# parthjaggi/flow

Measured on AMD Instinct MI355X. Metric: env-steps/sec, higher is better.
Workload: dtype mixed

## Files before the change

flow_amd/csrc/flowsim.hip:

```cpp
#include "flowsim_sim.h"
#include "flowsim_learn.h"
#include "flowsim_es.h"

#include <cmath>

namespace fsim {

int validate(const fs_config* c) {
  if (!c) return fail(FS_ERR_INVALID, "fs_create: cfg is NULL");
  if (c->struct_size != sizeof(fs_config))
    return fail(FS_ERR_INVALID, "fs_create: struct_size mismatch (header/library out of sync)");
  if (c->abi_version != FS_ABI_VERSION) return fail(FS_ERR_INVALID, "fs_create: abi_version mismatch");
  if (c->precision != FS_F32 && c->precision != FS_F64 && c->precision != FS_MIXED && c->precision != FS_F16S)
    return fail(FS_ERR_INVALID, "fs_create: bad precision");
  if (c->precision == FS_F16S && (c->network != FS_NET_MERGE || c->num_vehicles > 64))
    return fail(FS_ERR_UNSUPPORTED, "fs_create: FS_F16S (half state, float32 integrator) is built for FS_NET_MERGE "
                                    "(k_steps_open, <= 64 vehicle slots)");
  if (c->precision == FS_MIXED && (c->network == FS_NET_MERGE || c->network == FS_NET_BOTTLENECK)) {
  } else if (c->precision == FS_MIXED) {
    const bool fig8 = c->network == FS_NET_FIGURE_EIGHT;
    const char* why = nullptr;
    if ((c->network != FS_NET_RING && !fig8) || c->num_lanes > 1) why = "network (single-lane ring or figure eight)";
    else if (c->env == FS_ENV_MULTI_WAVE_ATTENUATION_PO)
      why = "env (FS_ENV_MULTI_WAVE_ATTENUATION_PO is built for FS_F32, and for FS_F64 on the generic kernel)";
// ... 251 lines not shown
  s->seg = seg;
  hipError_t e = hipSetDevice(cfg->device);
  if (e == hipSuccess) e = hipStreamCreateWithFlags(&s->own_stream, hipStreamNonBlocking);
  if (e != hipSuccess) {
    delete s;
    return fail(FS_ERR_HIP, std::string("fs_create: no usable HIP device: ") + hipGetErrorString(e));
  }
  s->stream = s->own_stream;
  {
    const std::pair<const char*, bool SimBase::*> switches[] = {
        {"FLOWSIM_FORCE_GENERIC", &SimBase::force_generic}, {"FLOWSIM_NO_FASTDIV", &SimBase::no_fastdiv},
        {"FLOWSIM_NO_LOOP_KERNEL", &SimBase::no_loop_kernel}, {"FLOWSIM_NO_LOOP_FULL", &SimBase::no_loop_full},
        {"FLOWSIM_NO_RING_RL", &SimBase::no_ring_rl}, {"FLOWSIM_NO_QUEUE", &SimBase::no_queue},
        {"FLOWSIM_NO_PAIR", &SimBase::no_pair}, {"FLOWSIM_PAIR_GENERIC_N", &SimBase::pair_generic_n},
        {"FLOWSIM_KERNEL_DETAIL", &SimBase::kernel_detail}, {"FLOWSIM_PAIR_N_ALWAYS", &SimBase::pair_n_always},
        {"FLOWSIM_NO_MASK_SKIP", &SimBase::no_mask_skip},
        {"FLOWSIM_SNAPSHOT_COPIES", &SimBase::snap_copies}};
    for (const auto& sw : switches) {
      const char* v = std::getenv(sw.first);
      s->*sw.second = v && v[0] == '1';
    }
  }
  int rc = s->init();
  if (rc == FS_OK) {
    hipError_t e2 = hipStreamSynchronize(s->stream);
    if (e2 != hipSuccess) rc = fail(FS_ERR_HIP, std::string("fs_create: ") + hipGetErrorString(e2));
  }
  if (rc != FS_OK) {
    for (void* p : s->allocs) (void)hipFree(p);
    (void)hipStreamDestroy(s->own_stream);
// ... 779 lines not shown
```

flow_amd/csrc/flowsim_launch.h:

```cpp
#pragma once
#include "flowsim_sim.h"
#ifdef FS_PART_QUEUE
#include "flowsim_queue.h"
#include "flowsim_dropq.h"
#endif

namespace fsim {

#ifdef FS_PART_QUEUE
  template <typename T>
  int Sim<T>::launch_queue(const StepArgs& a) {
    const bool po = dv.env == FS_ENV_MERGE_PO;
    const bool noise = (dv.flags & fs::FLAG_HAS_NOISE) != 0, act = a.actions != nullptr && (po || ov.ma_apply_actions != 0);
    const auto k = pick(noise, [&](auto NZ) {
      return pick(act, [&](auto ACT) {
        return pick(po, [&](auto PO) { return &fs::k_merge_queue<NZ, ACT, false, PO>; });
      });
    });
    last_kernel = "k_merge_queue";
    hipLaunchKernelGGL(k, dim3(dv.R), dim3(64), 0, stream, dv, ov, qc, a.num_steps, a.actions, a.act_stride, a.obs, a.rew,
                       a.done, a.obs_every_step, fs::PolicyView{}, static_cast<float*>(nullptr), static_cast<float*>(nullptr),
                       0);
    return launched();
  }
// ... 159 lines not shown
  int Sim<T>::launch_obs_mixed(const StepArgs& a) {
    if constexpr (std::is_same<T, double>::value) {
      const int n = dv.R * dv.N;
      last_kernel = "k_obs_mixed";
      hipLaunchKernelGGL((fs::k_obs_mixed<T>), dim3((n + 255) / 256), dim3(256), 0, stream, dv, a.obs);
      return launched();
    } else {
      return fail(FS_ERR_UNSUPPORTED, "k_obs_mixed is a float64 kernel");
    }
  }

  template <typename T>
  template <int SEG>
  int Sim<T>::launch_pair(const StepArgs& a) {
    constexpr int ROW = SEG >= 16 ? SEG / 2 : 8;
    const bool fd = fastdiv_ok(), bc = neg_speed_possible, sm = speed_mode_any;
    const bool noise = std::is_same<T, float>::value && (dv.flags & fs::FLAG_HAS_NOISE);
    auto clamped = [&](auto SM, auto NZ) {
      return delta4 && fd && !bc ? &fs::k_rollout_pair<T, ROW, true, true, false, SM, NZ>
                                 : &fs::k_rollout_pair<T, ROW, false, false, true, SM, NZ>;
    };
    decltype(&fs::k_rollout_pair<T, ROW, false, false, true>) k = nullptr;
    if (noise) {
      if constexpr (std::is_same<T, float>::value) k = pick(sm, [&](auto SM) { return clamped(SM, std::true_type()); });
    } else if (sm) {
      k = clamped(std::true_type(), std::false_type());
    } else {
      k = pick(bc, [&](auto BC) {
        return delta4 && fd ? &fs::k_rollout_pair<T, ROW, true, true, BC>
                            : delta4 ? &fs::k_rollout_pair<T, ROW, true, false, BC> : &fs::k_rollout_pair<T, ROW, false, false, BC>;
      });
    }
    last_kernel = noise ? (sm ? "k_rollout_pair+speed_mode+noise" : "k_rollout_pair+noise")
                        : (sm ? "k_rollout_pair+speed_mode" : "k_rollout_pair");
    const int waves = (dv.R + (64 / ROW) - 1) / (64 / ROW);
    if constexpr (SEG == 32) {
      if (dv.N == 22 && delta4 && fd && !bc && !pair_generic_n && (a.num_steps >= PAIR_N_MIN_STEPS || pair_n_always)) {
        decltype(&fs::k_rollout_pair_n<T, 11>) kn = nullptr;
        if constexpr (std::is_same<T, float>::value) {
          kn = pick(sm, [&](auto SM) { return pick(noise, [&](auto NZ) { return &fs::k_rollout_pair_n<T, 11, SM, NZ>; }); });
        } else {
          kn = pick(sm, [&](auto SM) { return &fs::k_rollout_pair_n<T, 11, SM>; });
        }
        if (kernel_detail)
          last_kernel = noise ? (sm ? "k_rollout_pair+speed_mode+noise[n11]" : "k_rollout_pair+noise[n11]")
                              : (sm ? "k_rollout_pair+speed_mode[n11]" : "k_rollout_pair[n11]");
        hipLaunchKernelGGL(kn, dim3((waves + 3) / 4), dim3(256), 0, stream, dv, a.num_steps, a.obs, a.rew, a.done);
        return launched();
      }
    }
    hipLaunchKernelGGL(k, dim3((waves + 3) / 4), dim3(256), 0, stream, dv, a.num_steps, a.obs, a.rew, a.done);
    return launched();
  }

  template <typename T>
  template <int SEG>
  int Sim<T>::launch_idm(const StepArgs& a) {
    constexpr int RPW = 64 / SEG;
    const bool fd = fastdiv_ok();
    const auto k = pick(neg_speed_possible, [&](auto BC) {
      return delta4 && fd ? &fs::k_rollout_idm<T, SEG, true, true, BC>
                          : delta4 ? &fs::k_rollout_idm<T, SEG, true, false, BC> : &fs::k_rollout_idm<T, SEG, false, false, BC>;
    });
    last_kernel = "k_rollout_idm";
    const int waves = (dv.R + RPW - 1) / RPW;
    hipLaunchKernelGGL(k, dim3((waves + 7) / 8), dim3(512), 0, stream, dv, a.num_steps, a.obs, a.rew, a.done, d_dump);
    return launched();
// ... 125 lines not shown
```

flow_amd/csrc/flowsim_pair.h:

```cpp
#pragma once
#include "flowsim_kernels.h"

namespace fs {

typedef float f2 __attribute__((ext_vector_type(2)));
typedef unsigned u2v __attribute__((__vector_size__(8)));

enum : int { DPP_ROW_NEWBCAST0 = 0x150, DPP_ROW_NEWBCAST8 = 0x158 };

__device__ __forceinline__ f2 fma2(f2 a, f2 b, f2 c) { return __builtin_elementwise_fma(a, b, c); }
__device__ __forceinline__ f2 splat(float a) { return f2{a, a}; }

__device__ __forceinline__ f2 pk_mul(f2 a, f2 b) { return a * b; }
__device__ __forceinline__ f2 pk_add(f2 a, f2 b) { return a + b; }
__device__ __forceinline__ f2 pk_sub(f2 a, f2 b) { return a - b; }
__device__ __forceinline__ f2 pk_fma(f2 a, f2 b, f2 c) { return fma2(a, b, c); }
__device__ __forceinline__ f2 pk_fnma(f2 a, f2 b, f2 c) { return fma2(-a, b, c); }
__device__ __forceinline__ float nonneg_else(float x, float y) {
  const unsigned a = __builtin_bit_cast(unsigned, x), b = __builtin_bit_cast(unsigned, y);
  return __builtin_bit_cast(float, min(a, b));
}

template <int ROW>
__device__ __forceinline__ float next_a(float v, bool last, int lane) {
// ... 149 lines not shown
      "v_fma_f64 v[130:131], -v[134:135], %[ms], v[130:131]\n"
      "v_fma_f64 v[132:133], -v[136:137], %[ms], v[132:133]\n"
      "v_fma_f64 v[134:135], v[130:131], %[rcms], v[134:135]\n"
      "v_fma_f64 v[136:137], v[132:133], %[rcms], v[136:137]\n"
      "v_cvt_f32_f64_e32 v128, v[134:135]\n"
      "v_cvt_f32_f64_e32 v129, v[136:137]\n"
      : "+{v[112:113]}"(V), "+{v[114:115]}"(X), "+{v[116:117]}"(H), "+{v[118:119]}"(DVL), "={v[128:129]}"(OV),
        [cb] "+v"(crash_bits), [sq] "=&v"(sq)
      : [L2] "v"(c.L2), [lenlead] "v"(c.len_lead), [gap2] "v"(c.gap2), [vmask] "v"(c.vmask), [tvm] "v"(c.tvm),
        [ms] "v"(c.ms64), [rcms] "v"(c.rc_ms64), [last] "s"(c.last_mask)
      : "v124", "v125", "v126", "v127", "v130", "v131", "v132", "v133", "v134", "v135", "v136", "v137");
}

struct MixedConsts {
  f2 p0, p1, p2, p5, rc_v0, tsab, rc_ab, one, gap2, vmask, tvm;
  float c1e3;
  double dt, ramp, L, rc_L, rc_ms, len_b, len_next, zero;
  unsigned L_lo, L_hi, thr;
  unsigned long long last_mask;
};
__device__ __forceinline__ void mixed_step_asm_a(f2& V32, double& XA, double& XB, double& VA, double& VB, f2& H, f2& DVL,
                                                 f2& OV, const MixedConsts& c) {
  asm volatile(
      "v_pk_mul_f32 v[124:125], v[112:113], v[142:143]\n"
      "v_pk_mul_f32 v[126:127], v[124:125], %[rcab]\n"
      "v_pk_fma_f32 v[130:131], v[126:127], %[tsab], v[124:125] neg_lo:[1,0,0] neg_hi:[1,0,0]\n"
      "v_pk_fma_f32 v[126:127], v[130:131], %[rcab], v[126:127]\n"
      "v_pk_mul_f32 v[124:125], v[112:113], %[rcv0]\n"
      "v_rcp_f32_e32 v122, v140\n"
      "v_rcp_f32_e32 v123, v141\n"
      "v_pk_fma_f32 v[130:131], v[124:125], %[p0], v[112:113] neg_lo:[1,0,0] neg_hi:[1,0,0]\n"
// ... 148 lines not shown
      "v_mul_f64 v[122:123], v[138:139], %[rcms]\n"
      "v_cvt_f32_f64_e32 v128, v[120:121]\n"
      "v_cvt_f32_f64_e32 v129, v[122:123]\n"
      : "+{v[112:113]}"(V32), "+{v[114:115]}"(XA), "+{v[116:117]}"(XB), "+{v[118:119]}"(VA), "+{v[138:139]}"(VB),
        "+{v[140:141]}"(H), "+{v[142:143]}"(DVL), "={v[128:129]}"(OV)
      : [c1e3] "v"(c.c1e3), [rcab] "v"(c.rc_ab), [tsab] "v"(c.tsab), [rcv0] "v"(c.rc_v0), [p0] "v"(c.p0),
        [p1] "v"(c.p1), [p2] "v"(c.p2), [p5] "v"(c.p5), [one] "v"(c.one), [dt] "v"(c.dt), [ramp] "v"(c.ramp),
        [rcms] "v"(c.rc_ms), [zero] "v"(c.zero), [rcts] "v"(m.rc_ts), [ts] "v"(m.ts),
        [rcsm] "v"(m.rc_smax), [smax] "v"(m.smax), [tau] "v"(m.tau), [mgap] "v"(m.min_gap), [maxa] "v"(m.maxa),
        [fl0a] "v"(d.fl0a), [fl0b] "v"(d.fl0b), [adta] "v"(d.adta), [adtb] "v"(d.adtb), [ddta] "v"(d.ddta),
        [ddtb] "v"(d.ddtb)
      : "v120", "v121", "v122", "v123", "v124", "v125", "v126", "v127", "v130", "v131", "v132", "v133", "v134",
        "v135", "v136", "v137", "v146", "v147", "v148", "v149", "v150", "v151", "v152", "v153", "v154", "v155");
}
__device__ __forceinline__ void mixed_step_asm_b(f2& V32, double& XA, double& XB, f2& H, f2& DVL, f2& OX, const double& WA,
                                                 const double& WB, float& ct, float& sq, unsigned long long& need,
                                                 const MixedConsts& c) {
  asm volatile(
      "v_sub_f32_e32 v142, v112, v113\n"
      "v_subrev_f32_dpp v143, v112, v113 row_shl:1 row_mask:0xf bank_mask:0xf bound_ctrl:1\n"
      "v_subrev_f32_dpp v124, v112, v113 row_newbcast:0 row_mask:0xf bank_mask:0xf\n"
      "v_mov_b32_dpp v130, v114 row_shl:1 row_mask:0xf bank_mask:0xf bound_ctrl:1\n"
      "v_mov_b32_dpp v131, v115 row_shl:1 row_mask:0xf bank_mask:0xf bound_ctrl:1\n"
      "v_mov_b32_dpp v132, v114 row_newbcast:0 row_mask:0xf bank_mask:0xf\n"
      "v_mov_b32_dpp v133, v115 row_newbcast:0 row_mask:0xf bank_mask:0xf\n"
      "v_add_f64 v[134:135], v[116:117], -v[114:115]\n"
      "v_cndmask_b32_e64 v130, v130, v132, %[last]\n"
      "v_cndmask_b32_e64 v131, v131, v133, %[last]\n"
      "v_add_f64 v[134:135], v[134:135], %[wa]\n"
      "v_add_f64 v[136:137], v[130:131], -v[116:117]\n"
      "v_cndmask_b32_e64 v143, v143, v124, %[last]\n"
      "v_add_f64 v[120:121], v[134:135], -%[lenb]\n"
      "v_add_f64 v[136:137], v[136:137], %[wb]\n"
      "v_max3_u32 v126, v115, v117, v135\n"
      "v_add_f64 v[122:123], v[136:137], -%[lennext]\n"
      "v_cvt_f32_f64_e32 v140, v[120:121]\n"
      "v_cvt_f32_f64_e32 v141, v[122:123]\n"
      "v_min_f32_e32 v127, v140, v141\n"
      "v_sub_u32_e32 v125, v127, %[c1e3]\n"
      "v_max3_u32 v126, v126, v137, v125\n"
      "v_cmp_le_u32_e64 %[need], %[thr], v126\n"
      "v_mul_f64 v[120:121], v[114:115], %[rcL]\n"
      "v_mul_f64 v[122:123], v[116:117], %[rcL]\n"
      "v_pk_fma_f32 v[124:125], v[112:113], %[vmask], %[tvm]\n"
      "v_cvt_f32_f64_e32 v144, v[120:121]\n"
      "v_cvt_f32_f64_e32 v145, v[122:123]\n"
      "v_pk_mul_f32 v[124:125], v[124:125], v[124:125]\n"
      "v_sub_f32_e32 %[ct], v127, %[gap]\n"
      "v_add_f32_e32 %[sq], v124, v125\n"
      : "+{v[112:113]}"(V32), "+{v[114:115]}"(XA), "+{v[116:117]}"(XB), "+{v[140:141]}"(H), "+{v[142:143]}"(DVL),
        "=&{v[144:145]}"(OX), [ct] "=&v"(ct), [sq] "=&v"(sq), [need] "=&s"(need)
      : [wa] "{v[156:157]}"(WA), [wb] "{v[158:159]}"(WB), [rcL] "v"(c.rc_L), [gap] "v"(c.gap2.x), [vmask] "v"(c.vmask), [tvm] "v"(c.tvm),
        [lenb] "v"(c.len_b), [lennext] "v"(c.len_next), [c1e3] "v"(c.c1e3), [thr] "v"(c.thr), [last] "s"(c.last_mask)
      : "v120", "v121", "v122", "v123", "v124", "v125", "v126", "v127", "v130", "v131", "v132", "v133", "v134", "v135",
        "v136", "v137");
}
__device__ __forceinline__ void mixed_step_asm_slow(double& XA, double& XB, f2& H, f2& OX, double& WA, double& WB, float& ct,
                                                    const MixedConsts& c) {
  unsigned long long sa, sb;
  asm volatile(
      "v_add_f64 v[134:135], v[114:115], -%[L]\n"
      "v_add_f64 v[136:137], v[116:117], -%[L]\n"
      "v_cmp_gt_i32_e64 %[sa], 0, v135\n"
      "v_cmp_gt_i32_e64 %[sb], 0, v137\n"
      "s_nop 0\n"
      "v_cndmask_b32_e64 v114, v134, v114, %[sa]\n"
      "v_cndmask_b32_e64 v115, v135, v115, %[sa]\n"
      "v_cndmask_b32_e64 v116, v136, v116, %[sb]\n"
// ... 21 lines not shown
      "v_add_f64 v[134:135], v[134:135], -%[lenb]\n"
      "v_cvt_f32_f64_e32 v140, v[134:135]\n"
      "v_cndmask_b32_e64 v136, v136, v132, %[sb]\n"
      "v_cndmask_b32_e64 v137, v137, v133, %[sb]\n"
      "v_cndmask_b32_e64 v158, 0, %[Llo], %[sb]\n"
      "v_cndmask_b32_e64 v159, 0, %[Lhi], %[sb]\n"
      "v_add_f64 v[136:137], v[136:137], -%[lennext]\n"
      "v_cvt_f32_f64_e32 v141, v[136:137]\n"
      "v_pk_add_f32 v[126:127], v[140:141], %[gap2] neg_lo:[0,1] neg_hi:[0,1]\n"
      "v_cmp_nlt_f32_e64 %[sa], |v140|, %[c1e3]\n"
      "v_cmp_nlt_f32_e64 %[sb], |v141|, %[c1e3]\n"
      "v_min_f32_e32 %[ct], v126, v127\n"
      "v_cndmask_b32_e64 v140, %[c1e3], v140, %[sa]\n"
      "v_cndmask_b32_e64 v141, %[c1e3], v141, %[sb]\n"
      : "+{v[114:115]}"(XA), "+{v[116:117]}"(XB), "+{v[140:141]}"(H), "+{v[144:145]}"(OX), "+{v[156:157]}"(WA),
        "+{v[158:159]}"(WB), [ct] "+v"(ct), [sa] "=&s"(sa), [sb] "=&s"(sb)
      : [L] "v"(c.L), [Llo] "v"(c.L_lo), [Lhi] "v"(c.L_hi), [rcL] "v"(c.rc_L), [gap2] "v"(c.gap2), [lenb] "v"(c.len_b),
        [lennext] "v"(c.len_next), [c1e3] "v"(c.c1e3), [last] "s"(c.last_mask)
      : "v120", "v121", "v122", "v123", "v126", "v127", "v130", "v131", "v132", "v133", "v134", "v135", "v136", "v137");
}

template <typename F, int... S>
__device__ __forceinline__ void each_slot(F&& f, std::integer_sequence<int, S...>) {
  (f(std::integral_constant<int, S>()), ...);
}

template <typename T, int ROW, bool DELTA4, bool FASTDIV, bool BADCHK, bool SM, bool NOISE, int NH>
__device__ __forceinline__ void rollout_pair_body(const DevView<T>& s, int num_steps, float* __restrict__ obs,
                                                  float* __restrict__ rew, uint8_t* __restrict__ done) {
  constexpr bool MIXED = sizeof(T) == 8;
  static_assert(!(NOISE && MIXED), "FS_MIXED has no noise form (its C twin cannot reproduce the hardware's log / cos)");
// ... 32 lines not shown
      gauss4<float>(s.seed_lo, s.seed_hi, s.rep0 + uint32_t(rr), uint32_t(iA), nctr >> 2, gA, s.noise_exact != 0);
      gauss4<float>(s.seed_lo, s.seed_hi, s.rep0 + uint32_t(rr), uint32_t(iB), nctr >> 2, gB, s.noise_exact != 0);
      for (uint32_t q = 0; q < (nctr & 3u); ++q) {
        gA[0] = gA[1]; gA[1] = gA[2]; gA[2] = gA[3];
        gB[0] = gB[1]; gB[1] = gB[2]; gB[2] = gB[3];
      }
    }
  }

  const float dt = float(s.dt), ramp = float(s.ramp);
  const f2 two_sqrt_ab = {2.0f * tsqrt(p[2].x * p[3].x), 2.0f * tsqrt(p[2].y * p[3].y)};
  const f2 rc_v0 = {1.0f / p[0].x, 1.0f / p[0].y}, rc_ab = {1.0f / two_sqrt_ab.x, 1.0f / two_sqrt_ab.y};
  const float Lf = float(L);
  const f2 L2 = splat(Lf), rc_L2 = splat(1.0f / Lf), one = splat(1.0f), dt2 = splat(dt), ramp2 = splat(ramp);
  const f2 gap2 = splat(float(s.crash_gap)), m100 = splat(-100.0f);
  const f2 vmask = splat(valid ? 1.0f : 0.0f), tvm = splat(valid ? -float(s.target_velocity) : 0.0f);
  const double ms64 = double(s.max_speed), rc_ms64 = 1.0 / ms64;
  const double L64 = double(L), rc_L64 = 1.0 / L64, dt64 = double(s.dt), ramp64 = double(s.ramp);

  f2 x, v;
  double xdA = 0, xdB = 0, vdA = 0, vdB = 0;
  if (MIXED) {
    xdA = double(s.pos[idx]); xdB = double(s.pos[idx + 1]);
    vdA = double(s.vel[idx]); vdB = double(s.vel[idx + 1]);
    v = f2{float(vdA), float(vdB)};
    x = f2{0.0f, 0.0f};
  } else {
    x = f2{float(s.pos[idx]), float(s.pos[idx + 1])};
    v = f2{float(s.vel[idx]), float(s.vel[idx + 1])};
  }
  const f2 len_lead = {float(lenB), float(len_nextA)};
// ... 18 lines not shown
  f2 vl = {v.y, next_a<ROW>(v.x, last, lane)};
  f2 dvl = v - vl;
  PairConsts pc;
  pc.p0 = p[0]; pc.p1 = p[1]; pc.p2 = p[2]; pc.p5 = p[5]; pc.rc_v0 = rc_v0; pc.tsab = two_sqrt_ab; pc.rc_ab = rc_ab;
  pc.one = one; pc.dt2 = dt2; pc.ramp2 = ramp2; pc.L2 = L2; pc.rc_L2 = rc_L2; pc.len_lead = len_lead;
  pc.gap2 = gap2; pc.vmask = vmask; pc.tvm = tvm; pc.c1e3 = 1e-3f; pc.ms64 = ms64; pc.rc_ms64 = rc_ms64;
  pc.last_mask = __ballot(last);
  MixedConsts mc;
  mc.p0 = p[0]; mc.p1 = p[1]; mc.p2 = p[2]; mc.p5 = p[5]; mc.rc_v0 = rc_v0; mc.tsab = two_sqrt_ab; mc.rc_ab = rc_ab;
  mc.one = one; mc.gap2 = gap2; mc.vmask = vmask; mc.tvm = tvm; mc.c1e3 = 1e-3f; mc.dt = dt64; mc.ramp = ramp64;
  mc.L = L64; mc.rc_L = rc_L64; mc.rc_ms = rc_ms64; mc.len_b = double(lenB); mc.len_next = double(len_nextA);
  mc.zero = 0.0; mc.last_mask = pc.last_mask;
  {
    const unsigned long long Lb = __builtin_bit_cast(unsigned long long, L64);
    mc.L_lo = unsigned(Lb); mc.L_hi = unsigned(Lb >> 32);
    mc.thr = mc.L_hi < 0x457CED91u ? mc.L_hi : 0x457CED91u;
  }
  double wA = 0.0, wB = 0.0;
  if constexpr (ASM && MIXED) {
    asm volatile("" : "+v"(mc.dt), "+v"(mc.ramp), "+v"(mc.one), "+v"(mc.zero), "+v"(mc.rc_ms), "+v"(mc.c1e3), "+v"(mc.gap2));
    const double xn = next_a<ROW>(xdA, last, lane);
    wA = xdB - xdA < 0.0 ? L64 : 0.0;
    wB = xn - xdB < 0.0 ? L64 : 0.0;
    h.x = tabs(h.x) < 1e-3f ? 1e-3f : h.x;
    h.y = tabs(h.y) < 1e-3f ? 1e-3f : h.y;
  }
  SumoPair sc{};
  double floor0A = 0, floor0B = 0, adtA = 0, adtB = 0, ddtA = 0, ddtB = 0;
  if constexpr (SM) {
    const int mA = s.speed_mode[iA], mB = s.speed_mode[iB];
    const float maA = float(s.max_accel[iA]), maB = float(s.max_accel[iB]);
    const float mdA = float(s.max_decel[iA]), mdB = float(s.max_decel[iB]);
    sc.tau = f2{float(s.sumo_tau[iA]), float(s.sumo_tau[iB])};
    sc.min_gap = f2{float(s.sumo_min_gap[iA]), float(s.sumo_min_gap[iB])};
    sc.maxa = f2{maA, maB};
// ... 101 lines not shown
        if (fresh) {
          gauss4<float>(s.seed_lo, s.seed_hi, s.rep0 + uint32_t(rr), uint32_t(iA), nctr >> 2, gA, s.noise_exact != 0);
          gauss4<float>(s.seed_lo, s.seed_hi, s.rep0 + uint32_t(rr), uint32_t(iB), nctr >> 2, gB, s.noise_exact != 0);
        }
      }
      const float tA = sigma.x * gA[0], tB = sigma.y * gB[0];
      nz.x = noisyA ? tA : -0.0f;
      nz.y = noisyB ? tB : -0.0f;
      gA[0] = gA[1]; gA[1] = gA[2]; gA[2] = gA[3];
      gB[0] = gB[1]; gB[1] = gB[2]; gB[2] = gB[3];
      nctr += 1u;
    }
    return nz;
  };

  auto one_step = [&](int slot, __amdgpu_buffer_rsrc_t rs, float& sq_out, auto IN_RING, __amdgpu_buffer_rsrc_t rs_prev)
                      __attribute__((always_inline)) {
    if constexpr (ASM) {
      f2 ov, ox;
      const unsigned so = unsigned(slot) * step_b32;
      auto store_late = [&]() {
        if constexpr (decltype(IN_RING)::value) {
          if (!BURST && slot >= 1 && slot <= NPIECE) __builtin_amdgcn_raw_buffer_store_b128(piece, rs_prev, doff[slot - 1], 0, 0);
        } else {
          if (slot > 0) __builtin_amdgcn_raw_buffer_store_b128(piece, rs, off_16, so - step_b32, 0);
        }
      };
      auto rows_in = [&]() {
        if constexpr (decltype(IN_RING)::value) ring_in(slot, ov, ox);
        else transpose_in(ov, ox);
      };
      if constexpr (MIXED) {
        if constexpr (SM) mixed_step_asm_a_sm(v, xdA, xdB, vdA, vdB, h, dvl, ov, mc, sc, msc);
        else mixed_step_asm_a(v, xdA, xdB, vdA, vdB, h, dvl, ov, mc);
        store_late();
        float ct;
        unsigned long long need;
        mixed_step_asm_b(v, xdA, xdB, h, dvl, ox, wA, wB, ct, sq_out, need, mc);
#if defined(FS_DIAG_ALWAYS_SLOW)
        need = ~0ull;
#elif defined(FS_DIAG_NEVER_SLOW)
        need = 0ull;
#endif
        if (__builtin_expect(need != 0ull, 0)) mixed_step_asm_slow(xdA, xdB, h, ox, wA, wB, ct, mc);
        crash_bits = __builtin_amdgcn_alignbit(crash_bits, __builtin_bit_cast(unsigned, ct), 31);
        rows_in();
      } else {
#if defined(FS_DIAG_NOSTORE)
        pair_step_asm_a(v, x, h, dvl, ox, pc);
        pair_step_asm_b(v, x, h, dvl, ov, crash_bits, sq_out, pc);
        asm volatile("" :: "v"(ov), "v"(ox), "s"(so));
#elif defined(FS_DIAG_NOXPOSE)
        pair_step_asm_a(v, x, h, dvl, ox, pc);
        __builtin_amdgcn_raw_buffer_store_b64(__builtin_bit_cast(u2v, ox), rs, off_x, so, 0);
        pair_step_asm_b(v, x, h, dvl, ov, crash_bits, sq_out, pc);
        __builtin_amdgcn_raw_buffer_store_b64(__builtin_bit_cast(u2v, ov), rs, off_v, so, 0);
#else
        if constexpr (NOISE) {
          const f2 nz = noise_term();
          if constexpr (SM) pair_step_asm_a_sm_nz(v, x, h, dvl, ox, pc, sc, nz);
// ... 59 lines not shown
      const f2 vb = pk_sub(v, m100);
      bad_bits = __builtin_amdgcn_alignbit(bad_bits, __builtin_bit_cast(unsigned, __builtin_fminf(vb.x, vb.y)), 31);
    }
    f2 ov;
    if (MIXED) ov = f2{float(vdA * rc_ms64), float(vdB * rc_ms64)};
    else ov = f2{div_via_f64(v.x, ms64, rc_ms64), div_via_f64(v.y, ms64, rc_ms64)};
    const unsigned so = unsigned(slot) * step_b32;
    __builtin_amdgcn_raw_buffer_store_b64(__builtin_bit_cast(u2v, ov), rs, off_v, so, 0);
    __builtin_amdgcn_raw_buffer_store_b64(__builtin_bit_cast(u2v, ox), rs, off_x, so, 0);
    const f2 dv = pk_fma(v, vmask, tvm);
    const f2 sq = pk_mul(dv, dv);
    sq_out = sq.x + sq.y;
  };

  int base = 0;
  char* ob_prev = ob;
  unsigned prev_bytes = 0u;
  const std::integral_constant<bool, RING> in_ring{};
  for (; base + PERIOD <= num_steps; base += PERIOD) {
    float sq[PERIOD];
    const size_t remain = size_t(num_steps - base) * step_bytes;
    const __amdgpu_buffer_rsrc_t rs = __builtin_amdgcn_make_buffer_rsrc(
        ob, 0, remain > 0xFFFFFFFFull ? 0xFFFFFFFFu : unsigned(remain), 0x00020000);
    const __amdgpu_buffer_rsrc_t rs_prev = __builtin_amdgcn_make_buffer_rsrc(ob_prev, 0, prev_bytes, 0x00020000);
    if constexpr (RING) {
      each_slot([&](auto S) __attribute__((always_inline)) { one_step(S.value, rs, sq[S.value], in_ring, rs_prev); },
                std::make_integer_sequence<int, PERIOD>());
    } else {
#pragma unroll
      for (int slot = 0; slot < PERIOD; ++slot) one_step(slot, rs, sq[slot], in_ring, rs_prev);
    }
#if !defined(FS_DIAG_NOSTORE) && !defined(FS_DIAG_NOXPOSE)
    if constexpr (RING) {
      if constexpr (BURST) {
#pragma unroll
        for (int j = 0; j < NPIECE; ++j) __builtin_amdgcn_raw_buffer_store_b128(ring_piece(j), rs, doff[j], 0, 0);
        __builtin_amdgcn_fence(__ATOMIC_RELEASE, "wavefront");
        __builtin_amdgcn_wave_barrier();
        __builtin_amdgcn_fence(__ATOMIC_ACQUIRE, "wavefront");
      } else {
        ob_prev = ob;
        prev_bytes = unsigned(PERIOD) * step_b32;
      }
    } else if (XPOSE) {
      __builtin_amdgcn_raw_buffer_store_b128(piece, rs, off_16, unsigned(PERIOD - 1) * step_b32, 0);
    }
#endif
    ob += size_t(PERIOD) * step_bytes;
    tcount += PERIOD;
    const float racc = transposed_sum<ROW, PERIOD>(sq, lane);
    const unsigned crash_any = seg_or<ROW>(crash_bits);
    const unsigned bad_any = (BADCHK ? seg_or<ROW>(bad_bits) : 0u) | crash_any;
    crash_bits = 0u;
    bad_bits = 0u;
    if (rvalid && k < PERIOD) {
      const bool my_crash = (crash_any >> (PERIOD - 1 - k)) & 1u;
      const bool my_bad = (bad_any >> (PERIOD - 1 - k)) & 1u;
      const int t_k = tcount - (PERIOD - 1 - k);
      const float cost = tsqrt(racc);
      const float max_cost = float(s.max_cost);
      float reward = tmax(max_cost - cost, 0.0f) / (max_cost + 1.1920928955078125e-07f);
      reward = my_bad ? 0.0f : reward;
      const size_t o = size_t(base + k) * s.R + rr;
      rew[o] = reward;
      done[o] = done_flag(t_k >= s.step_limit, my_crash);
    }
  }
  if (RING && !BURST && prev_bytes != 0u) {
    const __amdgpu_buffer_rsrc_t rs_prev = __builtin_amdgcn_make_buffer_rsrc(ob_prev, 0, prev_bytes, 0x00020000);
#pragma unroll
    for (int j = 0; j < NPIECE; ++j) __builtin_amdgcn_raw_buffer_store_b128(ring_piece(j), rs_prev, doff[j], 0, 0);
    __builtin_amdgcn_fence(__ATOMIC_RELEASE, "wavefront");
    __builtin_amdgcn_wave_barrier();
    __builtin_amdgcn_fence(__ATOMIC_ACQUIRE, "wavefront");
  }
#pragma unroll 1
  for (; base < num_steps; ++base) {
    float sq1;
    const __amdgpu_buffer_rsrc_t rs = __builtin_amdgcn_make_buffer_rsrc(ob, 0, unsigned(step_bytes), 0x00020000);
    one_step(0, rs, sq1, std::false_type(), rs);
#if !defined(FS_DIAG_NOSTORE) && !defined(FS_DIAG_NOXPOSE)
    if (XPOSE) __builtin_amdgcn_raw_buffer_store_b128(piece, rs, off_16, 0u, 0);
#endif
    ob += step_bytes;
    tcount += 1;
    const float racc = seg_sum<ROW>(sq1);
    const bool my_crash = (seg_or<ROW>(crash_bits) & 1u) != 0u;
    const bool my_bad = (BADCHK && (seg_or<ROW>(bad_bits) & 1u) != 0u) || my_crash;
    crash_bits = 0u;
    bad_bits = 0u;
    if (rvalid && k == 0) {
      const float cost = tsqrt(racc);
      const float max_cost = float(s.max_cost);
      float reward = tmax(max_cost - cost, 0.0f) / (max_cost + 1.1920928955078125e-07f);
      reward = my_bad ? 0.0f : reward;
// ... 45 lines not shown
```

flow_amd/csrc/flowsim_sim.h:

```cpp
#pragma once
#include <hip/hip_runtime.h>

#include <algorithm>
#include <climits>
#include <cmath>
#include <cstdio>
#include <cstdlib>
#include <cstring>
#include <map>
#include <mutex>
#include <new>
#include <string>
#include <type_traits>
#include <vector>

#include "flowsim.h"
#include "flowsim_kernels.h"
#include "flowsim_open.h"
#include "flowsim_pair.h"
#include "flowsim_fig8.h"
#include "flowsim_ringrl.h"
#include "flowsim_policy.h"
#include "flowsim_wide.h"
#include "flowsim_queue_consts.h"
// ... 53 lines not shown
  float* d_obs = nullptr;
  float* d_rew = nullptr;
  uint8_t* d_done = nullptr;
  uint8_t* d_mask = nullptr;
  float* d_dump = nullptr;
  std::vector<void*> allocs;
  int after_reset = 0;
  bool force_generic = false;
  bool no_fastdiv = false;
  bool f16s = false;
  bool mixed = false;
  bool no_pair = false;
  bool pair_generic_n = false;
  bool pair_n_always = false;
  static constexpr int PAIR_N_MIN_STEPS = 512;
  bool kernel_detail = false;
  bool no_loop_kernel = false;
  bool no_loop_full = false;
  bool no_ring_rl = false;
  bool no_mask_skip = false;
  bool no_queue = false;
  bool snap_copies = false;
  double* d_ep_scratch = nullptr;
  double* d_adv_scratch = nullptr;
  unsigned* d_mb_ticket = nullptr;
  int* d_qflag = nullptr;
  bool qflag_armed = false;
  int check_qflag() {
    if (!qflag_armed || !d_qflag) return FS_OK;
    int f = 0;
// ... 369 lines not shown
    }
    return FS_OK;
  }

  std::vector<T> snap_ring_len;
  bool snap_out_stale = true;
  bool snap_in_stale = false;
  bool snap_neg = false, snap_init_neg = false;
  static void sorted_union(std::vector<T>& into, const std::vector<T>& more) {
    into.insert(into.end(), more.begin(), more.end());
    std::sort(into.begin(), into.end());
    into.erase(std::unique(into.begin(), into.end()), into.end());
  }
  void ring_mirror_changed() {
    fastdiv_state = -1;
    ringrl_fast_state = -1;
    snap_out_stale = true;
    snap_in_stale = true;
  }
  void snap_mirrors_out() override {
    if (snap_out_stale) {
      sorted_union(snap_ring_len, h_ring_len);
      snap_out_stale = false;
    }
    snap_neg = snap_neg || neg_speed_possible;
    snap_init_neg = snap_init_neg || init_vel_negative;
  }
  void snap_mirrors_in() override {
    if (snap_in_stale) {
      std::vector<T> have = h_ring_len;
      sorted_union(have, {});
      std::vector<T> all = have;
      sorted_union(all, snap_ring_len);
      if (all.size() != have.size()) {
        h_ring_len = all;
        fastdiv_state = -1;
        ringrl_fast_state = -1;
        snap_out_stale = true;
      }
      snap_in_stale = false;
    }
    neg_speed_possible = neg_speed_possible || snap_neg;
    init_vel_negative = init_vel_negative || snap_init_neg;
  }
  void snap_mirrors_blob(const char* dev_part) override {
    const size_t R = size_t(dv.R);
    for (int k = 0; k < snap.n; ++k) {
      const fs::SnapEntry& en = snap.e[k];
      const T* vals = reinterpret_cast<const T*>(dev_part + en.off);
      const size_t count = R * en.row / sizeof(T);
      if (en.tag == fs::SNAP_RING_LEN || en.tag == fs::SNAP_INIT_RING_LEN) {
// ... 267 lines not shown
  bool fastdiv_ok() {
    if ((!std::is_same<T, float>::value && !mixed) || force_generic || no_fastdiv) return false;
    return prove_divisors(fastdiv_state, [&](std::vector<float>& cs) {
      for (int i = 0; i < dv.N; ++i) {
        add_idm_divisors(cs, i);
        if (!gap_in(veh[i].p[5], 1e-3f)) return false;
        if (speed_mode_any) {
          add_sumo_divisors(cs, i);
          if (!gap_in(veh[i].sumo_min_gap, 1e-3f)) return false;
        }
      }
      return add_ring_divisors(cs, 80);
    });
  }

  int loop_fastc_state = -1;
  bool loop_fastc_ok() {
    if (!(std::is_same<T, float>::value || mixed) || no_fastdiv) return false;
    return prove_divisors(loop_fastc_state, [&](std::vector<float>& cs) {
      if (!loop_div_ok) return false;
      for (int i = 0; i < dv.N; ++i) {
        if (veh[i].controller == FS_CTRL_IDM) add_idm_divisors(cs, i);
        add_sumo_divisors(cs, i);
      }
      return true;
    });
  }

  int ringrl_fast_state = -1;
  bool ringrl_fast_ok() {
// ... 651 lines not shown
```

Measured before the change: 14.79 billion.

## Move crash-gap check into slow path and compute pair rewards inline

In the mixed-precision pair kernel, the crash-gap comparison is folded into the fast-path need threshold. The crash bit is then computed only inside the rarely taken slow path, which removes a subtract and an alignbit from every step. Reward and done outputs are written by every lane through buffer stores with running offsets, and the per-block resource rebuilding from remaining bytes is simplified. Host-side guards (pair_gap_ok) prove the threshold folding is valid, and launches are split into chunks so that 32-bit buffer offsets do not overflow. The cost is extra kernel launches for very long rollouts and more complex correctness conditions.

```diff
diff --git a/flow_amd/csrc/flowsim.hip b/flow_amd/csrc/flowsim.hip
--- a/flow_amd/csrc/flowsim.hip
+++ b/flow_amd/csrc/flowsim.hip
@@ -289,6 +289,7 @@
         {"FLOWSIM_NO_RING_RL", &SimBase::no_ring_rl}, {"FLOWSIM_NO_QUEUE", &SimBase::no_queue},
         {"FLOWSIM_NO_PAIR", &SimBase::no_pair}, {"FLOWSIM_PAIR_GENERIC_N", &SimBase::pair_generic_n},
         {"FLOWSIM_KERNEL_DETAIL", &SimBase::kernel_detail}, {"FLOWSIM_PAIR_N_ALWAYS", &SimBase::pair_n_always},
+        {"FLOWSIM_PAIR_SPLIT", &SimBase::pair_split},
         {"FLOWSIM_NO_MASK_SKIP", &SimBase::no_mask_skip},
         {"FLOWSIM_SNAPSHOT_COPIES", &SimBase::snap_copies}};
     for (const auto& sw : switches) {
diff --git a/flow_amd/csrc/flowsim_launch.h b/flow_amd/csrc/flowsim_launch.h
--- a/flow_amd/csrc/flowsim_launch.h
+++ b/flow_amd/csrc/flowsim_launch.h
@@ -197,7 +197,7 @@
   template <int SEG>
   int Sim<T>::launch_pair(const StepArgs& a) {
     constexpr int ROW = SEG >= 16 ? SEG / 2 : 8;
-    const bool fd = fastdiv_ok(), bc = neg_speed_possible, sm = speed_mode_any;
+    const bool fd = fastdiv_ok() && (!mixed || pair_gap_ok()), bc = neg_speed_possible, sm = speed_mode_any;
     const bool noise = std::is_same<T, float>::value && (dv.flags & fs::FLAG_HAS_NOISE);
     auto clamped = [&](auto SM, auto NZ) {
       return delta4 && fd && !bc ? &fs::k_rollout_pair<T, ROW, true, true, false, SM, NZ>
@@ -217,6 +217,21 @@
     last_kernel = noise ? (sm ? "k_rollout_pair+speed_mode+noise" : "k_rollout_pair+noise")
                         : (sm ? "k_rollout_pair+speed_mode" : "k_rollout_pair");
     const int waves = (dv.R + (64 / ROW) - 1) / (64 / ROW);
+    const int max_steps = pair_split ? 16 : int(std::min<size_t>(size_t(INT_MAX), ((size_t(1) << 30) - 1) / size_t(dv.R)) & ~size_t(15));
+    auto launch_split = [&](auto kern) {
+      float* o = a.obs;
+      float* r = a.rew;
+      uint8_t* d = a.done;
+      for (int left = a.num_steps; left > 0;) {
+        const int n = std::min(left, max_steps);
+        hipLaunchKernelGGL(kern, dim3((waves + 3) / 4), dim3(256), 0, stream, dv, n, o, r, d);
+        o += size_t(n) * dv.R * 2 * dv.N;
+        r += size_t(n) * dv.R;
+        d += size_t(n) * dv.R;
+        left -= n;
+      }
+      return launched();
+    };
     if constexpr (SEG == 32) {
       if (dv.N == 22 && delta4 && fd && !bc && !pair_generic_n && (a.num_steps >= PAIR_N_MIN_STEPS || pair_n_always)) {
         decltype(&fs::k_rollout_pair_n<T, 11>) kn = nullptr;
@@ -228,12 +243,10 @@
         if (kernel_detail)
           last_kernel = noise ? (sm ? "k_rollout_pair+speed_mode+noise[n11]" : "k_rollout_pair+noise[n11]")
                               : (sm ? "k_rollout_pair+speed_mode[n11]" : "k_rollout_pair[n11]");
-        hipLaunchKernelGGL(kn, dim3((waves + 3) / 4), dim3(256), 0, stream, dv, a.num_steps, a.obs, a.rew, a.done);
-        return launched();
-      }
-    }
-    hipLaunchKernelGGL(k, dim3((waves + 3) / 4), dim3(256), 0, stream, dv, a.num_steps, a.obs, a.rew, a.done);
-    return launched();
+        return launch_split(kn);
+      }
+    }
+    return launch_split(k);
   }
 
   template <typename T>
diff --git a/flow_amd/csrc/flowsim_pair.h b/flow_amd/csrc/flowsim_pair.h
--- a/flow_amd/csrc/flowsim_pair.h
+++ b/flow_amd/csrc/flowsim_pair.h
@@ -187,7 +187,7 @@
 
 struct MixedConsts {
   f2 p0, p1, p2, p5, rc_v0, tsab, rc_ab, one, gap2, vmask, tvm;
-  float c1e3;
+  float c1e3, cneed;
   double dt, ramp, L, rc_L, rc_ms, len_b, len_next, zero;
   unsigned L_lo, L_hi, thr;
   unsigned long long last_mask;
@@ -366,7 +366,7 @@
         "v135", "v136", "v137", "v146", "v147", "v148", "v149", "v150", "v151", "v152", "v153", "v154", "v155");
 }
 __device__ __forceinline__ void mixed_step_asm_b(f2& V32, double& XA, double& XB, f2& H, f2& DVL, f2& OX, const double& WA,
-                                                 const double& WB, float& ct, float& sq, unsigned long long& need,
+                                                 const double& WB, float& sq, unsigned long long& need,
                                                  const MixedConsts& c) {
   asm volatile(
       "v_sub_f32_e32 v142, v112, v113\n"
@@ -389,7 +389,7 @@
       "v_cvt_f32_f64_e32 v140, v[120:121]\n"
       "v_cvt_f32_f64_e32 v141, v[122:123]\n"
       "v_min_f32_e32 v127, v140, v141\n"
-      "v_sub_u32_e32 v125, v127, %[c1e3]\n"
+      "v_sub_u32_e32 v125, v127, %[cneed]\n"
       "v_max3_u32 v126, v126, v137, v125\n"
       "v_cmp_le_u32_e64 %[need], %[thr], v126\n"
       "v_mul_f64 v[120:121], v[114:115], %[rcL]\n"
@@ -398,12 +398,11 @@
       "v_cvt_f32_f64_e32 v144, v[120:121]\n"
       "v_cvt_f32_f64_e32 v145, v[122:123]\n"
       "v_pk_mul_f32 v[124:125], v[124:125], v[124:125]\n"
-      "v_sub_f32_e32 %[ct], v127, %[gap]\n"
       "v_add_f32_e32 %[sq], v124, v125\n"
       : "+{v[112:113]}"(V32), "+{v[114:115]}"(XA), "+{v[116:117]}"(XB), "+{v[140:141]}"(H), "+{v[142:143]}"(DVL),
-        "=&{v[144:145]}"(OX), [ct] "=&v"(ct), [sq] "=&v"(sq), [need] "=&s"(need)
-      : [wa] "{v[156:157]}"(WA), [wb] "{v[158:159]}"(WB), [rcL] "v"(c.rc_L), [gap] "v"(c.gap2.x), [vmask] "v"(c.vmask), [tvm] "v"(c.tvm),
-        [lenb] "v"(c.len_b), [lennext] "v"(c.len_next), [c1e3] "v"(c.c1e3), [thr] "v"(c.thr), [last] "s"(c.last_mask)
+        "=&{v[144:145]}"(OX), [sq] "=&v"(sq), [need] "=&s"(need)
+      : [wa] "{v[156:157]}"(WA), [wb] "{v[158:159]}"(WB), [rcL] "v"(c.rc_L), [vmask] "v"(c.vmask), [tvm] "v"(c.tvm),
+        [lenb] "v"(c.len_b), [lennext] "v"(c.len_next), [cneed] "v"(c.cneed), [thr] "v"(c.thr), [last] "s"(c.last_mask)
       : "v120", "v121", "v122", "v123", "v124", "v125", "v126", "v127", "v130", "v131", "v132", "v133", "v134", "v135",
         "v136", "v137");
 }
@@ -455,7 +454,7 @@
       "v_cndmask_b32_e64 v140, %[c1e3], v140, %[sa]\n"
       "v_cndmask_b32_e64 v141, %[c1e3], v141, %[sb]\n"
       : "+{v[114:115]}"(XA), "+{v[116:117]}"(XB), "+{v[140:141]}"(H), "+{v[144:145]}"(OX), "+{v[156:157]}"(WA),
-        "+{v[158:159]}"(WB), [ct] "+v"(ct), [sa] "=&s"(sa), [sb] "=&s"(sb)
+        "+{v[158:159]}"(WB), [ct] "=&v"(ct), [sa] "=&s"(sa), [sb] "=&s"(sb)
       : [L] "v"(c.L), [Llo] "v"(c.L_lo), [Lhi] "v"(c.L_hi), [rcL] "v"(c.rc_L), [gap2] "v"(c.gap2), [lenb] "v"(c.len_b),
         [lennext] "v"(c.len_next), [c1e3] "v"(c.c1e3), [last] "s"(c.last_mask)
       : "v120", "v121", "v122", "v123", "v126", "v127", "v130", "v131", "v132", "v133", "v134", "v135", "v136", "v137");
@@ -518,7 +517,8 @@
   const float Lf = float(L);
   const f2 L2 = splat(Lf), rc_L2 = splat(1.0f / Lf), one = splat(1.0f), dt2 = splat(dt), ramp2 = splat(ramp);
   const f2 gap2 = splat(float(s.crash_gap)), m100 = splat(-100.0f);
-  const f2 vmask = splat(valid ? 1.0f : 0.0f), tvm = splat(valid ? -float(s.target_velocity) : 0.0f);
+  const bool counted = k < LP;
+  const f2 vmask = splat(counted ? 1.0f : 0.0f), tvm = splat(counted ? -float(s.target_velocity) : 0.0f);
   const double ms64 = double(s.max_speed), rc_ms64 = 1.0 / ms64;
   const double L64 = double(L), rc_L64 = 1.0 / L64, dt64 = double(s.dt), ramp64 = double(s.ramp);
 
@@ -567,11 +567,14 @@
   {
     const unsigned long long Lb = __builtin_bit_cast(unsigned long long, L64);
     mc.L_lo = unsigned(Lb); mc.L_hi = unsigned(Lb >> 32);
-    mc.thr = mc.L_hi < 0x457CED91u ? mc.L_hi : 0x457CED91u;
+    mc.cneed = gap2.x > 1e-3f ? gap2.x : 1e-3f;
+    const unsigned tc = 0x80000000u - __builtin_bit_cast(unsigned, mc.cneed);
+    mc.thr = mc.L_hi < tc ? mc.L_hi : tc;
   }
   double wA = 0.0, wB = 0.0;
   if constexpr (ASM && MIXED) {
-    asm volatile("" : "+v"(mc.dt), "+v"(mc.ramp), "+v"(mc.one), "+v"(mc.zero), "+v"(mc.rc_ms), "+v"(mc.c1e3), "+v"(mc.gap2));
+    asm volatile("" : "+v"(mc.dt), "+v"(mc.ramp), "+v"(mc.one), "+v"(mc.zero), "+v"(mc.rc_ms), "+v"(mc.c1e3), "+v"(mc.gap2),
+                 "+v"(mc.cneed));
     const double xn = next_a<ROW>(xdA, last, lane);
     wA = xdB - xdA < 0.0 ? L64 : 0.0;
     wB = xn - xdB < 0.0 ? L64 : 0.0;
@@ -703,8 +706,8 @@
     return nz;
   };
 
-  auto one_step = [&](int slot, __amdgpu_buffer_rsrc_t rs, float& sq_out, auto IN_RING, __amdgpu_buffer_rsrc_t rs_prev)
-                      __attribute__((always_inline)) {
+  auto one_step = [&](int slot, __amdgpu_buffer_rsrc_t rs, float& sq_out, auto IN_RING, __amdgpu_buffer_rsrc_t rs_prev,
+                      int cbit) __attribute__((always_inline)) {
     if constexpr (ASM) {
       f2 ov, ox;
       const unsigned so = unsigned(slot) * step_b32;
@@ -723,16 +726,18 @@
         if constexpr (SM) mixed_step_asm_a_sm(v, xdA, xdB, vdA, vdB, h, dvl, ov, mc, sc, msc);
         else mixed_step_asm_a(v, xdA, xdB, vdA, vdB, h, dvl, ov, mc);
         store_late();
-        float ct;
         unsigned long long need;
-        mixed_step_asm_b(v, xdA, xdB, h, dvl, ox, wA, wB, ct, sq_out, need, mc);
+        mixed_step_asm_b(v, xdA, xdB, h, dvl, ox, wA, wB, sq_out, need, mc);
 #if defined(FS_DIAG_ALWAYS_SLOW)
         need = ~0ull;
 #elif defined(FS_DIAG_NEVER_SLOW)
         need = 0ull;
 #endif
-        if (__builtin_expect(need != 0ull, 0)) mixed_step_asm_slow(xdA, xdB, h, ox, wA, wB, ct, mc);
-        crash_bits = __builtin_amdgcn_alignbit(crash_bits, __builtin_bit_cast(unsigned, ct), 31);
+        if (__builtin_expect(need != 0ull, 0)) {
+          float ct;
+          mixed_step_asm_slow(xdA, xdB, h, ox, wA, wB, ct, mc);
+          crash_bits |= (__builtin_bit_cast(unsigned, ct) >> 31) << cbit;
+        }
         rows_in();
       } else {
 #if defined(FS_DIAG_NOSTORE)
@@ -822,21 +827,39 @@
   };
 
   int base = 0;
-  char* ob_prev = ob;
-  unsigned prev_bytes = 0u;
   const std::integral_constant<bool, RING> in_ring{};
-  for (; base + PERIOD <= num_steps; base += PERIOD) {
+  constexpr bool TAIL = ASM && PERIOD == ROW;
+  const float max_cost_f = float(s.max_cost);
+  const double mce64 = double(max_cost_f + 1.1920928955078125e-07f), rc_mce64 = 1.0 / mce64;
+  int hz_k = 0;
+  unsigned off_rew = 0u, off_done = 0u;
+  unsigned so_rew = 0u, so_done = 0u;
+  const unsigned rs_steps = TAIL ? unsigned(num_steps > 0 ? num_steps : 0) * unsigned(s.R) : 0u;
+  const __amdgpu_buffer_rsrc_t rs_rew = __builtin_amdgcn_make_buffer_rsrc(rew, 0, rs_steps * 4u, 0x00020000);
+  const __amdgpu_buffer_rsrc_t rs_done = __builtin_amdgcn_make_buffer_rsrc(done, 0, rs_steps, 0x00020000);
+  if constexpr (TAIL) {
+    long long hz = (long long)s.step_limit - (long long)tcount - (long long)k - 1ll;
+    hz = hz > 0x7FFFFFFFll ? 0x7FFFFFFFll : hz < -0x80000000ll ? -0x80000000ll : hz;
+    hz_k = int(hz);
+    off_done = unsigned(k) * unsigned(s.R) + unsigned(rr);
+    off_rew = off_done * 4u;
+  }
+  const unsigned blk_bytes = unsigned(PERIOD) * step_b32;
+  const int last_base = num_steps - PERIOD;
+#pragma unroll 1
+  for (; base <= last_base; base += PERIOD) {
     float sq[PERIOD];
-    const size_t remain = size_t(num_steps - base) * step_bytes;
-    const __amdgpu_buffer_rsrc_t rs = __builtin_amdgcn_make_buffer_rsrc(
-        ob, 0, remain > 0xFFFFFFFFull ? 0xFFFFFFFFu : unsigned(remain), 0x00020000);
-    const __amdgpu_buffer_rsrc_t rs_prev = __builtin_amdgcn_make_buffer_rsrc(ob_prev, 0, prev_bytes, 0x00020000);
+    const bool hz_blk = TAIL && base >= hz_k;
+    const __amdgpu_buffer_rsrc_t rs = __builtin_amdgcn_make_buffer_rsrc(ob, 0, blk_bytes, 0x00020000);
+    const __amdgpu_buffer_rsrc_t rs_prev = __builtin_amdgcn_make_buffer_rsrc(
+        reinterpret_cast<char*>(reinterpret_cast<uintptr_t>(ob) - blk_bytes), 0, base != 0 ? blk_bytes : 0u, 0x00020000);
     if constexpr (RING) {
-      each_slot([&](auto S) __attribute__((always_inline)) { one_step(S.value, rs, sq[S.value], in_ring, rs_prev); },
-                std::make_integer_sequence<int, PERIOD>());
+      each_slot([&](auto S) __attribute__((always_inline)) {
+        one_step(S.value, rs, sq[S.value], in_ring, rs_prev, PERIOD - 1 - S.value);
+      }, std::make_integer_sequence<int, PERIOD>());
     } else {
 #pragma unroll
-      for (int slot = 0; slot < PERIOD; ++slot) one_step(slot, rs, sq[slot], in_ring, rs_prev);
+      for (int slot = 0; slot < PERIOD; ++slot) one_step(slot, rs, sq[slot], in_ring, rs_prev, PERIOD - 1 - slot);
     }
 #if !defined(FS_DIAG_NOSTORE) && !defined(FS_DIAG_NOXPOSE)
     if constexpr (RING) {
@@ -846,9 +869,6 @@
         __builtin_amdgcn_fence(__ATOMIC_RELEASE, "wavefront");
         __builtin_amdgcn_wave_barrier();
         __builtin_amdgcn_fence(__ATOMIC_ACQUIRE, "wavefront");
-      } else {
-        ob_prev = ob;
-        prev_bytes = unsigned(PERIOD) * step_b32;
       }
     } else if (XPOSE) {
       __builtin_amdgcn_raw_buffer_store_b128(piece, rs, off_16, unsigned(PERIOD - 1) * step_b32, 0);
@@ -861,7 +881,16 @@
     const unsigned bad_any = (BADCHK ? seg_or<ROW>(bad_bits) : 0u) | crash_any;
     crash_bits = 0u;
     bad_bits = 0u;
-    if (rvalid && k < PERIOD) {
+    if constexpr (TAIL) {
+      const bool my_crash = (crash_any & (1u << (PERIOD - 1 - k))) != 0u;
+      const float cost = tsqrt(racc);
+      float reward = div_via_f64(tmax(max_cost_f - cost, 0.0f), mce64, rc_mce64);
+      reward = my_crash ? 0.0f : reward;
+      __builtin_amdgcn_raw_buffer_store_b32(__builtin_bit_cast(unsigned, reward), rs_rew, off_rew, so_rew, 0);
+      __builtin_amdgcn_raw_buffer_store_b8(done_flag(hz_blk, my_crash), rs_done, off_done, so_done, 0);
+      so_rew += unsigned(PERIOD) * unsigned(s.R) * 4u;
+      so_done += unsigned(PERIOD) * unsigned(s.R);
+    } else if (rvalid && k < PERIOD) {
       const bool my_crash = (crash_any >> (PERIOD - 1 - k)) & 1u;
       const bool my_bad = (bad_any >> (PERIOD - 1 - k)) & 1u;
       const int t_k = tcount - (PERIOD - 1 - k);
@@ -874,8 +903,9 @@
       done[o] = done_flag(t_k >= s.step_limit, my_crash);
     }
   }
-  if (RING && !BURST && prev_bytes != 0u) {
-    const __amdgpu_buffer_rsrc_t rs_prev = __builtin_amdgcn_make_buffer_rsrc(ob_prev, 0, prev_bytes, 0x00020000);
+  if (RING && !BURST && base != 0) {
+    const __amdgpu_buffer_rsrc_t rs_prev = __builtin_amdgcn_make_buffer_rsrc(
+        reinterpret_cast<char*>(reinterpret_cast<uintptr_t>(ob) - blk_bytes), 0, blk_bytes, 0x00020000);
 #pragma unroll
     for (int j = 0; j < NPIECE; ++j) __builtin_amdgcn_raw_buffer_store_b128(ring_piece(j), rs_prev, doff[j], 0, 0);
     __builtin_amdgcn_fence(__ATOMIC_RELEASE, "wavefront");
@@ -886,7 +916,7 @@
   for (; base < num_steps; ++base) {
     float sq1;
     const __amdgpu_buffer_rsrc_t rs = __builtin_amdgcn_make_buffer_rsrc(ob, 0, unsigned(step_bytes), 0x00020000);
-    one_step(0, rs, sq1, std::false_type(), rs);
+    one_step(0, rs, sq1, std::false_type(), rs, 0);
 #if !defined(FS_DIAG_NOSTORE) && !defined(FS_DIAG_NOXPOSE)
     if (XPOSE) __builtin_amdgcn_raw_buffer_store_b128(piece, rs, off_16, 0u, 0);
 #endif
diff --git a/flow_amd/csrc/flowsim_sim.h b/flow_amd/csrc/flowsim_sim.h
--- a/flow_amd/csrc/flowsim_sim.h
+++ b/flow_amd/csrc/flowsim_sim.h
@@ -91,6 +91,7 @@
   bool pair_generic_n = false;
   bool pair_n_always = false;
   static constexpr int PAIR_N_MIN_STEPS = 512;
+  bool pair_split = false;
   bool kernel_detail = false;
   bool no_loop_kernel = false;
   bool no_loop_full = false;
@@ -490,6 +491,7 @@
   }
   void ring_mirror_changed() {
     fastdiv_state = -1;
+    pair_gap_state = -1;
     ringrl_fast_state = -1;
     snap_out_stale = true;
     snap_in_stale = true;
@@ -511,6 +513,7 @@
       if (all.size() != have.size()) {
         h_ring_len = all;
         fastdiv_state = -1;
+        pair_gap_state = -1;
         ringrl_fast_state = -1;
         snap_out_stale = true;
       }
@@ -808,6 +811,25 @@
     });
   }
 
+  int pair_gap_state = -1;
+  bool pair_gap_ok() {
+    if (pair_gap_state >= 0) return pair_gap_state == 1;
+    pair_gap_state = 0;
+    const float gap = float(cfg.crash_gap), mce = float(dv.max_cost) + 1.1920928955078125e-07f;
+    if (!(gap == gap) || !std::isnormal(mce) || !(mce > 0.0f)) return false;
+    const float c = gap > 1e-3f ? gap : 1e-3f;
+    uint32_t cb;
+    std::memcpy(&cb, &c, 4);
+    for (T b : h_ring_len) {
+      const double L = double(b) + 4.0 * double(dv.jlen);
+      uint64_t Lb;
+      std::memcpy(&Lb, &L, 8);
+      if (!(L > 0.0) || cb > 0x80000000u - uint32_t(Lb >> 32)) return false;
+    }
+    pair_gap_state = 1;
+    return true;
+  }
+
   int loop_fastc_state = -1;
   bool loop_fastc_ok() {
     if (!(std::is_same<T, float>::value || mixed) || no_fastdiv) return false;
```

Result: slower. 14.53 billion (-1.7%).
